# davrempe/contact-human-dynamics

Measured on NVIDIA H100. Metric: optimised frames/sec (batched phys-optim), higher is better.
Workload: dtype f64

## Files before the change

contact-human-dynamics_b200/csrc/chd_api.cu:

```cuda
#include <cuda_runtime.h>

#include <cstdio>
#include <cstdlib>
#include <cstring>
#include <vector>

#include "../../include/chd.h"
#include "chd_dev.h"

__global__ void chd_k_stage_begin(ChdDev D);
__global__ void chd_k_eval(ChdDev D);
__global__ void chd_k_init(ChdDev D);
__global__ void chd_k_kkt(ChdDev D);
__global__ void chd_k_kkt_gwin(ChdDev D);
__global__ void chd_k_kcopy(ChdDev D);
__global__ void chd_k_curv(ChdDev D);
__global__ void chd_k_asm(ChdDev D);
__global__ void chd_k_fp64_peak(int mode, int iters, double* sink);
__global__ void chd_k_hess_base(ChdDev D);
__global__ void chd_k_hess_dur(ChdDev D);
__global__ void chd_k_hess_zero(ChdDev D);
__global__ void chd_k_hess_fin(ChdDev D, int mode);
__global__ void chd_k_tables(ChdDev D);
__global__ void chd_k_clear_dyn(ChdDev D);
// ... 257 lines not shown
    CHD_CUDA(cudaGetDevice(&dev_id));
    CHD_CUDA(cudaDeviceGetDefaultMemPool(&pool, dev_id));
    unsigned long long keep = ~0ull;
    CHD_CUDA(cudaMemPoolSetAttribute(pool, cudaMemPoolAttrReleaseThreshold, &keep));
  }
  CHD_CUDA(cudaStreamCreateWithFlags(&b->copy_stream, cudaStreamNonBlocking));
  CHD_CUDA(cudaEventCreateWithFlags(&b->ev_kkt, cudaEventDisableTiming));
  CHD_CUDA(cudaEventCreateWithFlags(&b->ev_copy, cudaEventDisableTiming));
  CHD_CUDA(cudaEventCreateWithFlags(&b->ev_ls, cudaEventDisableTiming));
  CHD_CUDA(cudaEventCreate(&b->ev0));
  CHD_CUDA(cudaEventCreate(&b->ev1));
#define UP(field) if ((rc = dev_upload(b, hb.field, &D.field))) return rc;
#define UPM(field, T) if ((rc = dev_upload(b, hb.field, (const T**)&D.field))) return rc;
  UP(seq) UPM(poly_T, double) UPM(poly_tend, double) UP(node_const) UP(par) UP(t_dyn) UP(t_rom) UP(t_data) UP(row_lo) UP(row_hi) UP(node_var)
  UP(itab) UP(ent_ptr) UPM(ent_col, int) UP(ent_row) UP(col_ptr) UP(col_ent) UP(var_kkt) UP(row_kkt) UP(row_set) UP(sets) UPM(phase_tend, double)
  UP(dur0) UP(poly_ph)
  if ((rc = dev_upload(b, hb.poly_T, (const double**)&b->poly_T0))) return rc;
  if ((rc = dev_upload(b, hb.poly_tend, (const double**)&b->poly_tend0))) return rc;
  if ((rc = dev_upload(b, hb.phase_tend, (const double**)&b->phase_tend0))) return rc;
  if ((rc = dev_upload(b, hb.ent_col, (const int**)&b->ent_col0))) return rc;
  if ((rc = dev_upload(b, hb.poly_T, (const double**)&D.poly_Tt))) return rc;
  if ((rc = dev_upload(b, hb.poly_tend, (const double**)&D.poly_tendt))) return rc;
#undef UPM
#undef UP
  const size_t B = hb.B, nm = B * hb.n_max, mm = B * hb.m_max;
#define AL(field, cnt) if ((rc = dev_alloc(b, (cnt), &D.field))) return rc;
  AL(x, nm) AL(xt, nm) AL(jty, nm) AL(unobs, nm) AL(dx, nm) AL(grad, nm) AL(g, mm) AL(gt, mm) AL(Jv, B * hb.slots_max) AL(rflag, mm)
  AL(sc, mm) AL(dL, mm) AL(dU, mm) AL(s, mm) AL(y, mm) AL(zL, mm) AL(zU, mm) AL(ds, mm) AL(dy, mm) AL(dzL, mm) AL(dzU, mm)
  int dev = 0, sms = 0, smem_max = 0;
  CHD_CUDA(cudaGetDevice(&dev));
  CHD_CUDA(cudaDeviceGetAttribute(&sms, cudaDevAttrMultiProcessorCount, dev));
// ... 125 lines not shown

int chd_phys_get_layout(const chd_phys_batch* b, int32_t* ent_ptr, int32_t* ent_col, double* row_lo, double* row_hi,
                        int32_t* row_set, int32_t* var_kkt, int32_t* row_kkt) {
  if (!b) return -1;
  const ChdHostBatch& hb = b->hb;
  if (ent_ptr) std::memcpy(ent_ptr, hb.ent_ptr.data(), hb.ent_ptr.size() * sizeof(int));
  if (ent_col) std::memcpy(ent_col, hb.ent_col.data(), hb.ent_col.size() * sizeof(int));
  if (row_lo) std::memcpy(row_lo, hb.row_lo.data(), hb.row_lo.size() * sizeof(double));
  if (row_hi) std::memcpy(row_hi, hb.row_hi.data(), hb.row_hi.size() * sizeof(double));
  if (row_set) std::memcpy(row_set, hb.row_set.data(), hb.row_set.size() * sizeof(int));
  if (var_kkt) std::memcpy(var_kkt, hb.var_kkt.data(), hb.var_kkt.size() * sizeof(int));
  if (row_kkt) std::memcpy(row_kkt, hb.row_kkt.data(), hb.row_kkt.size() * sizeof(int));
  return 0;
}

int chd_phys_get_slot_index(const chd_phys_batch* b, int32_t* ent_row, int32_t* col_ptr, int32_t* col_ent) {
  if (!b) return -1;
  const ChdHostBatch& hb = b->hb;
  if (ent_row) std::memcpy(ent_row, hb.ent_row.data(), hb.ent_row.size() * sizeof(int));
  if (col_ptr) std::memcpy(col_ptr, hb.col_ptr.data(), hb.col_ptr.size() * sizeof(int));
  if (col_ent) std::memcpy(col_ent, hb.col_ent.data(), hb.col_ent.size() * sizeof(int));
  return 0;
}

int chd_phys_get_ent_col(const chd_phys_batch* b, int32_t* ent_col) {
  if (!b || !ent_col) return -1;
  if (b->host_only) {
    std::memcpy(ent_col, b->hb.ent_col.data(), b->hb.ent_col.size() * sizeof(int));
    return 0;
  }
// ... 139 lines not shown
```

contact-human-dynamics_b200/csrc/chd_dev.h:

```cpp
#pragma once
#include "chd_core.h"
#include "chd_kkt_plan.h"
#include "chd_layout.h"

#define CHD_FILT_MAX 24
#define CHD_THREADS 512
#define CHD_NL_GUARD 1.0
#define CHD_NL_FLOOR 1e-4
#define CHD_UNOBS_EPS 1e-14
#define CHD_DW_UNOBS 1e-4
#define CHD_CURV_MIN 1e-8

#define CHD_ROW_ACTIVE 1
#define CHD_ROW_EQ 2
#define CHD_ROW_HASL 4
#define CHD_ROW_HASU 8
#define CHD_ROW_WARM 16

#define CHD_PH_BEGIN 0
#define CHD_PH_RUN 1
#define CHD_PH_FINISHED 2
struct ChdIpm {
  int status;
  int iter, nfilt, ls_fail, max_iter, n_bounds, m_act, pad0;
// ... 25 lines not shown
  double w_data[3], w_vel[3], w_acc[3], w_dur;
};

struct ChdDev {
  int B, S, Pmax, n_max, m_max, slots_max, sets_max, tab_max, F_max, Kd_max, Kr_max, Na_max, nb_max, w_max, par_stride,
      n_ee_max, fo_max, Ph_max, win_smem, nbc_max, Q, Qfix, nbt, win_tiles, pan_doubles;
  size_t kstride;
  const ChdSeq* seq;
  double *poly_T, *poly_tend;
  const double *node_const, *par, *t_dyn, *t_rom, *t_data, *row_lo, *row_hi, *dur0;
  const int *node_var, *itab, *ent_ptr, *var_kkt, *row_kkt, *row_set, *poly_ph;
  int* ent_col;
  double *poly_Tt, *poly_tendt;
  double* jty;
  const int *ent_row, *col_ptr, *col_ent;
  const ChdSet* sets;
  double* phase_tend;
  double *x, *xt, *dx, *grad;
  double *g, *gt;
  double* Jv;
  int* rflag;
  unsigned char* unobs;
  double *sc, *dL, *dU, *s, *y, *zL, *zU, *ds, *dy, *dzL, *dzU;
  double* cost;
  double* Kwork;
  double* Kbase;
  double* sol;
  double* scratch;
  double *rhs0, *rhs1;
  size_t scratch_stride;
// ... 55 lines not shown
```

contact-human-dynamics_b200/csrc/chd_kkt.cu:

```cuda
#include <cuda_runtime.h>

#include "chd_block.cuh"
#include "chd_eval.cuh"
#include "chd_kkt_tiles.cuh"

__device__ __forceinline__ void chd_hess_sample(const ChdCtx& c, const ChdKT& K, const int* vk, int s, const ChdSpl* P, const double* sign, int np,
                                                int deriv, double wgt, int lane, double* ws) {
  const bool tau = c.opt_dur && s >= 2 && deriv == 0;
  if (lane < 28) {
    const int pa = lane / 14, q = lane % 14;
    double v0 = 0.0, v1 = 0.0, v2 = 0.0;
    int ia = -1;
    if (pa < np) {
      if (q < 12) {
        const int va = P[pa].var[q];
        const double wa = sign[pa] * chd_slot_w(P[pa], deriv, q);
        if (va >= 0 && wa != 0.0) {
          ia = vk[va];
          v0 = q % 3 == 0 ? wa : 0.0, v1 = q % 3 == 1 ? wa : 0.0, v2 = q % 3 == 2 ? wa : 0.0;
        }
      } else if (tau) {
        ChdTau u;
        chd_spl_tau(c, s, s - 2, P[pa], u);
        const int var = q == 12 ? u.va : u.vb;
// ... 7 lines not shown
  const int ne = np * 14;
  for (int idx = lane; idx < ne * ne; idx += 32) {
    const int a = idx / ne, bq = idx - a * ne;
    const int ia = (int)ws[a * 4], ib = (int)ws[bq * 4];
    if (ia < 0 || ib < 0 || ia < ib) continue;
    const double v = ws[a * 4 + 1] * ws[bq * 4 + 1] + ws[a * 4 + 2] * ws[bq * 4 + 2] + ws[a * 4 + 3] * ws[bq * 4 + 3];
    if (v != 0.0) chd_kadd(K, ia, ib, wgt * v);
  }
  __syncwarp();
}

__device__ void chd_hess_build(const ChdDev& D, int b, const ChdStageDev& sg, double* base, int part, int nparts) {
  const int tid = threadIdx.x, nt = blockDim.x;
  const ChdSeq* h = D.seq + b;
  ChdKT K;
  chd_kt_init(D, h, base, K);
  K.ovf = &D.ipm[b].band_ovf;
  const double sf = D.ipm[b].sf;
  const int* vk = D.var_kkt + (size_t)b * D.n_max;
  ChdCtx c;
  chd_make_ctx(D, b, D.x + (size_t)b * D.n_max, c);
  c.dyn = D.ipm[b].dyn;
  c.opt_dur = sg.opt_dur;
  const int n_ee = h->n_ee, nsp = 2 + n_ee, F = h->F, ns = h->n_smooth;
  __shared__ double s_hws[CHD_THREADS / 32][28 * 4];
  const int lane = tid & 31, warp = tid >> 5, nwarp = nt >> 5;
  for (int it = part * nwarp + warp; it < nsp * F; it += nparts * nwarp) {
    const int s = it / F, i = it % F, cls = s < 2 ? s : 2;
    ChdSpl P[2];
    double sgn[2] = {1.0, -1.0};
    chd_spl_at(c, s, c.t_data[i], P[1]);
// ... 42 lines not shown
}
__global__ void __launch_bounds__(128) chd_k_hess_fin(ChdDev D, int mode) {
  const int b = blockIdx.x;
  ChdIpm& I = D.ipm[b];
  double* base;
  if (mode == 0) {
    if (I.phase != CHD_PH_BEGIN) return;
    base = D.Kbase + (size_t)b * D.kstride;
  } else {
    if (I.phase != CHD_PH_RUN || !I.kw_req || !D.stages[I.stage].opt_dur) return;
    base = D.Kwork + (size_t)b * D.kstride;
  }
  const ChdSeq* h = D.seq + b;
  const int* vk = D.var_kkt + (size_t)b * D.n_max;
  ChdKT K;
  chd_kt_init(D, h, base, K);
  unsigned char* un = D.unobs + (size_t)b * D.n_max;
  const int mot_lo = h->sp_xoff[2], mot_hi = h->sp_xoff[2 + h->n_ee];
  for (int i = mot_lo + threadIdx.x; i < mot_hi; i += blockDim.x) {
    const int k = vk[i];
    un[i] = k >= 0 && *chd_kdiag(K, k) <= CHD_UNOBS_EPS;
  }
  __syncthreads();
  if (mode == 0 && threadIdx.x == 0) I.phase = CHD_PH_RUN;
}

__device__ __forceinline__ void chd_curv_rows(const ChdDev& D, int b, const ChdKT& K, const ChdStageDev& sg, int wid, int nw, int lane,
                                              double* ws) {
  const ChdSeq* h = D.seq + b;
  const size_t ro = (size_t)b * D.m_max, vo = (size_t)b * D.n_max;
  const int* vk = D.var_kkt + vo;
// ... 81 lines not shown
}

__global__ void __launch_bounds__(256) chd_k_hess_zero(ChdDev D) {
  const int b = blockIdx.y;
  if (D.ipm[b].phase != CHD_PH_BEGIN) return;
  chd_hess_clear(D, b, D.Kbase + (size_t)b * D.kstride, blockIdx.x, gridDim.x);
  chd_hess_clear(D, b, D.Kwork + (size_t)b * D.kstride, blockIdx.x, gridDim.x);
  if (blockIdx.x == 0) chd_rhs_clear(D, b);
}
__global__ void __launch_bounds__(256, 2) chd_k_hess_base(ChdDev D) {
  __shared__ double s_ws[8][192];
  const int b = blockIdx.y;
  if (D.ipm[b].phase != CHD_PH_BEGIN) return;
  const ChdStageDev sg = D.stages[D.ipm[b].stage];
  ChdKT K;
  chd_kt_init(D, D.seq + b, D.Kwork + (size_t)b * D.kstride, K);
  K.ovf = &D.ipm[b].band_ovf;
  const int warp = threadIdx.x >> 5, nwarp = blockDim.x >> 5;
  chd_curv_rows(D, b, K, sg, blockIdx.x * nwarp + warp, gridDim.x * nwarp, threadIdx.x & 31, s_ws[warp]);
  chd_hess_build(D, b, sg, D.Kbase + (size_t)b * D.kstride, blockIdx.x, gridDim.x);
  chd_hess_build(D, b, sg, D.Kwork + (size_t)b * D.kstride, blockIdx.x, gridDim.x);
}

__device__ __forceinline__ void chd_assemble(const ChdDev& D, int b, const ChdKT& K, double delta_w, double sf, int t0, int tstep,
                                             double* g0, double* g1) {
  const ChdSeq* h = D.seq + b;
  const int n = D.stages[D.ipm[b].stage].opt_dur ? h->n : h->n - h->n_dur;
  const int m = h->m, Na = K.Na;
  const size_t ro = (size_t)b * D.m_max, vo = (size_t)b * D.n_max;
  const int* rf = D.rflag + ro;
  const int* vk = D.var_kkt + vo;
// ... 97 lines not shown
  const int b = blockIdx.x;
  c.b = b, c.I = &I;
  c.sg = D.stages[I.stage];
  const ChdSeq* h = c.h = D.seq + b;
  c.n = h->n, c.m = h->m, c.tid = threadIdx.x, c.nt = blockDim.x;
  c.lane = c.tid & 31, c.warp = c.tid >> 5, c.nwarp = c.nt >> 5;
  c.ro = (size_t)b * D.m_max, c.vo = (size_t)b * D.n_max;
  c.rf = D.rflag + c.ro;
  c.vk = D.var_kkt + c.vo;
  c.rk = D.row_kkt + c.ro;
  c.ep = D.ent_ptr + (size_t)b * (D.m_max + 1);
  c.ec = D.ent_col + (size_t)b * D.slots_max;
  c.Jv = D.Jv + (size_t)b * D.slots_max;
  c.grad = D.grad + c.vo;
  ChdKT& K = c.K;
  chd_kt_init(D, h, D.Kwork + (size_t)b * D.kstride, K);
  K.ovf = &I.band_ovf;
  if (!c.sg.opt_dur) K.q = D.Qfix - 1;
  c.n_act = c.sg.opt_dur ? c.n : c.n - h->n_dur;
  c.Qs = K.Q, c.Q = c.sg.opt_dur ? K.Q : D.Qfix, c.nbt = K.nbt, c.nbp8 = K.nbp8, c.nbl = c.sg.opt_dur ? h->nb : h->nb_fix, c.nbc = K.nbc;
  c.NBR = c.nbl, c.nbt_s = (c.nbl + 1 + 7) >> 3;
  c.n_even = (size_t)((D.n_max + 1) & ~1), c.xs_len = (size_t)(8 * D.nbc_max + c.nbp8);
  double* gs = WS ? nullptr : D.scratch + (size_t)b * D.scratch_stride;
  c.red = sm;
  c.cc = c.red + CHD_KKT_THREADS;
  c.ypan = c.cc + c.nbp8 * c.nbp8;
  c.xpan = c.ypan + (c.Q + c.nbt) * 64;
  c.dinv = c.ypan + D.pan_doubles;
  c.win_region = (size_t)D.win_tiles * 64 + (size_t)c.Qs * c.nbt * 64;
  c.win = WS ? c.dinv + 16 : gs + c.n_even + c.xs_len + 8 * (size_t)D.nbc_max;
  c.bwin = c.win + (size_t)D.win_tiles * 64;
  c.vecn = WS ? c.win + c.win_region - c.n_even : gs;
  c.xs = WS ? c.vecn - c.xs_len : c.vecn + c.n_even;
// ... 248 lines not shown
        tl[i].C[r8] = c0[i], tl[i].C[r8 + 1] = c1[i];
      }
  }
}

template <bool WS>
__device__ __forceinline__ void chd_kkt_factor(const ChdKktCtx& c, int& s_fail) {
  const ChdKT& K = c.K;
  const int tid = c.tid, nt = c.nt, lane = c.lane, warp = c.warp, nwarp = c.nwarp;
  const int Qs = c.Qs, Q = c.Q, nbt = c.nbt, nbp8 = c.nbp8, nbc = c.nbc, nbt_s = c.nbt_s;
  double *cc = c.cc, *ypan = c.ypan, *xpan = c.xpan, *dinv = c.dinv, *win = c.win, *bwin = c.bwin;
  for (int i = tid; i < nbp8 * nbp8; i += nt) cc[i] = K.corn[i];
  if (WS) {
    for (int idx = tid; idx < Q * Q * 64; idx += nt) {
      const int e = idx & 63, pr = idx >> 6, J = pr / Q, t = pr % Q;
      if (J + t < Q && J < nbc && J + t < nbc) win[chd_win_slot(J + t, J, Q) * 64 + e] = K.band[((size_t)J * Qs + t) * 64 + e];
    }
    for (int idx = tid; idx < Q * nbt * 64; idx += nt) {
      const int J = idx / (nbt * 64);
      if (J < nbc) bwin[idx] = K.bord[(size_t)J * nbt * 64 + idx % (nbt * 64)];
    }
  }
  __syncthreads();
  __shared__ int s_rs[2][96];
  __shared__ int s_gnz[2][96];
  constexpr int kPairs = WS ? 3000 : CHD_KKT_GROUPS_MAX * (CHD_KKT_GROUPS_MAX + 1) / 2;
  __shared__ unsigned short s_pairs[kPairs];
  __shared__ unsigned char s_cmp[CHD_KKT_THREADS / 32][64];
  __shared__ __align__(16) double s_winv[2][64];
  const int GB = K.q, Gm = K.q + nbt_s, npairs = Gm * (Gm + 1) / 2;
  for (int p = tid; p < npairs && p < kPairs; p += nt) {
    int gi = (int)((sqrt(8.0 * p + 1.0) - 1.0) * 0.5);
    while (gi * (gi + 1) / 2 > p) --gi;
    while ((gi + 1) * (gi + 2) / 2 <= p) ++gi;
    s_pairs[p] = (unsigned short)((gi << 8) | (p - gi * (gi + 1) / 2));
  }
  auto tri = [](int a_, int b_) { return a_ > b_ ? a_ * (a_ + 1) / 2 + b_ : b_ * (b_ + 1) / 2 + a_; };
  for (int g = tid; g < GB; g += nt) s_rs[0][g] = (1 + g) % Q;
  for (int g = tid; g < 96; g += nt) s_gnz[0][g] = 0, s_gnz[1][g] = 0;
  if (warp == 0) {
    const bool ok = chd_tile_ldl(WS ? win : K.band, dinv, s_winv[0], lane);
    if (!ok && lane == 0) s_fail = 1;
  }
  __syncthreads();
  int kslot = 0, cur = 0;
  for (int Kc = 0; Kc < nbc; ++Kc, cur ^= 1) {
    const int tq = min(K.q, nbc - 1 - Kc);
    const int* rs = s_rs[cur];
    auto band_tile = [&](int gi, int gj) -> double* {
      return WS ? win + (size_t)tri(rs[gi], rs[gj]) * 64 : K.band + ((size_t)(Kc + 1 + gj) * Qs + (gi - gj)) * 64;
    };
    auto bord_tile = [&](int bi, int gj) -> double* {
      return WS ? bwin + ((size_t)rs[gj] * nbt + bi) * 64 : K.bord + ((size_t)(Kc + 1 + gj) * nbt + bi) * 64;
    };
    double* Tkk = WS ? win + (size_t)tri(kslot, kslot) * 64 : K.band + (size_t)Kc * Qs * 64;
    double* Bk = WS ? bwin + (size_t)kslot * nbt * 64 : K.bord + (size_t)Kc * nbt * 64;
    const double* dv = dinv + 8 * cur;
    {
      const double* wv = s_winv[cur];
      const int r = lane >> 2, k = lane & 3;
      const double2 wf = *reinterpret_cast<const double2*>(wv + 2 * lane);
      const double d0 = dv[2 * k], d1 = dv[2 * k + 1];
// ... 11 lines not shown
                     : "+d"(c0), "+d"(c1)
                     : "d"(ay), "d"(wf.y));
        const double x0 = c0 * d0, x1 = c1 * d1;
        ypan[pg * 64 + f0] = c0, ypan[pg * 64 + f1] = c1;
        xpan[pg * 64 + f0] = x0, xpan[pg * 64 + f1] = x1;
        double* G = band_t ? K.band + ((size_t)Kc * Qs + 1 + g) * 64 : K.bord + ((size_t)Kc * nbt + (g - tq)) * 64;
        *reinterpret_cast<double2*>(G + r * 8 + 2 * k) = make_double2(x0, x1);
        const bool nz = __any_sync(0xffffffffu, x0 != 0.0 || x1 != 0.0);
        if (lane == 0 && nz) s_gnz[cur][pg] = 1;
      }
    }
    if (WS)
      for (int e = tid; e < 64; e += nt) K.band[(size_t)Kc * Qs * 64 + e] = Tkk[e];
    __syncthreads();
    const int In = Kc + Q;
    if (WS && In < nbc) {
      for (int idx = tid - 32; idx < Q * 32 + nbt_s * 32; idx += nt - 32) {
        if (idx < 0) break;
        const int tile = idx >> 5, off = (idx & 31) * 2;
        if (tile < Q) {
          const int J = tile < GB ? Kc + 1 + tile : In;
          double* dst = tile < GB ? win + (size_t)tri(kslot, rs[tile]) * 64 : Tkk;
          chd_copy16(dst + off, K.band + ((size_t)J * Qs + (In - J)) * 64 + off, WS);
        } else {
          chd_copy16(Bk + (tile - Q) * 64 + off, K.bord + (size_t)In * nbt * 64 + (tile - Q) * 64 + off, WS);
        }
      }
    }
    if (warp == 0) {
      if (tq >= 1) {
        double* Tn = band_tile(0, 0);
        chd_tile_sub_xyT(Tn, xpan, ypan, lane);
        __syncwarp();
        const bool ok = chd_tile_ldl(Tn, dinv + 8 * (cur ^ 1), s_winv[cur ^ 1], lane);
        if (!ok && lane == 0) s_fail = 1;
      }
    } else {
      if (warp == 1) {
        for (int g = lane; g < GB; g += 32) {
          int v = kslot + 2 + g;
          while (v >= Q) v -= Q;
          s_rs[cur ^ 1][g] = v;
        }
        for (int g = lane; g < Gm; g += 32) s_gnz[cur ^ 1][g] = 0;
      }
      if (!WS && Gm > 64) chd_kkt_update_wide(c, s_pairs, s_gnz[cur], GB, npairs, tq, band_tile, bord_tile);
      else chd_kkt_update_compact(c, s_pairs, s_cmp[warp], s_gnz[cur], GB, Gm, tq, band_tile, bord_tile);
    }
// ... 47 lines not shown
    const double* bt = K.bord + (size_t)(i >> 3) * nbt * 64 + (i & 7);
    double v = bt[NBR * 8];
    for (int q2 = 0; q2 < nbl; ++q2) v -= bt[q2 * 8] * xb[q2];
    accv[i] = v;
  }
  const int per = Q * 64;
  const int R = max(1, (int)((c.win_region - (WS ? c.n_even + c.xs_len : 0)) / 64) / (2 * Q));
  double* stg = c.win;
  auto stage_chunk = [&](int Ktop, int buf, int t0, int tstep) {
    for (int idx = t0; idx < R * Q * 32; idx += tstep) {
      const int rr = idx / (Q * 32), rem = idx - rr * (Q * 32);
      const int Kr = Ktop - rr;
      if (Kr < 0) break;
      const int tile = rem >> 5, off = (rem & 31) * 2;
      const int J = tile == 0 ? Kr : Kr - tile;
      if (J < 0) continue;
      chd_copy16(stg + ((size_t)buf * R + rr) * per + tile * 64 + off, K.band + ((size_t)J * Qs + (Kr - J)) * 64 + off, WS);
    }
  };
  stage_chunk(nbc - 1, 0, tid, nt);
  chd_copy_wait(WS);
  __syncthreads();
  int buf = 0;
  for (int Ktop = nbc - 1; Ktop >= 0; Ktop -= R, buf ^= 1) {
    if (warp != 0) {
      stage_chunk(Ktop - R, buf ^ 1, tid - 32, nt - 32);
    } else {
      for (int rr = 0; rr < R && Ktop - rr >= 0; ++rr) {
        const int Kc = Ktop - rr;
        const double* T0 = stg + ((size_t)buf * R + rr) * per;
        double xk[8];
#pragma unroll
        for (int cl = 7; cl >= 0; --cl) {
          double v = accv[Kc * 8 + cl];
#pragma unroll
          for (int p = 7; p > cl; --p) v -= T0[p * 8 + cl] * xk[p];
          xk[cl] = v;
        }
        if (lane < 8) {
          const int gi = Kc * 8 + lane;
          double v = xk[0];
#pragma unroll
          for (int cl = 1; cl < 8; ++cl) v = lane == cl ? xk[cl] : v;
          xs[gi] = v;
          if (gi < Na) sol[gi] = v;
        }
        const int nrow = min(K.q, Kc);
        for (int idx = lane; idx < nrow * 8; idx += 32) {
          const int g = idx >> 3, cl = idx & 7;
          const double* T = T0 + (g + 1) * 64;
          double v = 0.0;
#pragma unroll
          for (int r = 0; r < 8; ++r) v += T[r * 8 + cl] * xk[r];
          accv[(Kc - 1 - g) * 8 + cl] -= v;
        }
        __syncwarp();
      }
    }
    chd_copy_wait(WS);
    __syncthreads();
  }
}
// ... 120 lines not shown
}
#undef CHD_PROF

__global__ void __launch_bounds__(256) chd_k_kcopy(ChdDev D) {
  const int b = blockIdx.y;
  if (!D.ipm[b].kw_req) return;
  if (blockIdx.x == 0) chd_rhs_clear(D, b);
  if (D.stages[D.ipm[b].stage].opt_dur && D.ipm[b].phase == CHD_PH_RUN) {
    chd_hess_clear(D, b, D.Kwork + (size_t)b * D.kstride, blockIdx.x, gridDim.x);
    return;
  }
  const size_t cnt2 = D.kstride / 2, per = (cnt2 + gridDim.x - 1) / gridDim.x;
  const size_t lo = (size_t)blockIdx.x * per, hi = lo + per < cnt2 ? lo + per : cnt2;
  const double2* src = reinterpret_cast<const double2*>(D.Kbase + (size_t)b * D.kstride);
  double2* dst = reinterpret_cast<double2*>(D.Kwork + (size_t)b * D.kstride);
  const size_t nt = blockDim.x;
  size_t i = lo + threadIdx.x;
  for (; i + 3 * nt < hi; i += 4 * nt) {
    const double2 v0 = src[i], v1 = src[i + nt], v2 = src[i + 2 * nt], v3 = src[i + 3 * nt];
    dst[i] = v0, dst[i + nt] = v1, dst[i + 2 * nt] = v2, dst[i + 3 * nt] = v3;
  }
  for (; i < hi; i += nt) dst[i] = src[i];
}

__global__ void __launch_bounds__(256) chd_k_curv(ChdDev D) {
  __shared__ double s_ws[8 * 192];
  const int b = blockIdx.y;
  const ChdIpm& I = D.ipm[b];
  if (!I.kw_req || I.phase != CHD_PH_RUN) return;
  ChdKT K;
  chd_kt_init(D, D.seq + b, D.Kwork + (size_t)b * D.kstride, K);
  K.ovf = &D.ipm[b].band_ovf;
  const int warp = threadIdx.x >> 5, lane = threadIdx.x & 31;
  chd_curv_rows(D, b, K, D.stages[I.stage], blockIdx.x * 8 + warp, gridDim.x * 8, lane, s_ws + warp * 192);
}

__global__ void __launch_bounds__(256) chd_k_asm(ChdDev D) {
  const int b = blockIdx.y;
  const ChdIpm& I = D.ipm[b];
  if (I.phase != CHD_PH_RUN) return;
  ChdKT K;
  chd_kt_init(D, D.seq + b, D.Kwork + (size_t)b * D.kstride, K);
  K.ovf = &D.ipm[b].band_ovf;
  if (!D.stages[I.stage].opt_dur) K.q = D.Qfix - 1;
  const size_t go = (size_t)b * (D.Na_max + D.nb_max);
  chd_assemble(D, b, K, I.delta_w, I.sf, blockIdx.x * blockDim.x + threadIdx.x, gridDim.x * blockDim.x, D.rhs0 + go, D.rhs1 + go);
}

__global__ void __launch_bounds__(256) chd_k_fp64_peak(int mode, int iters, double* sink) {
  const double s = 1.0 + 1e-9 * threadIdx.x;
  double a[8];
#pragma unroll
  for (int i = 0; i < 8; ++i) a[i] = 0.5 + i;
  if (mode == 0) {
    for (int it = 0; it < iters; ++it) {
#pragma unroll
      for (int i = 0; i < 8; ++i) a[i] = fma(a[i], s, 1e-3);
    }
  } else {
// ... 18 lines not shown
```

contact-human-dynamics_b200/csrc/chd_kkt_tiles.cuh:

```cuda
#pragma once
#include "chd_dev.h"

struct ChdKT {
  int Na, Np, nbc, q, Q, nbt, nbp8;
  double *band, *bord, *corn;
  int* ovf;
};

__device__ __forceinline__ void chd_kt_init(const ChdDev& D, const ChdSeq* h, double* base, ChdKT& K) {
  K.Na = h->Na;
  K.Np = (h->Na + 7) & ~7;
  K.nbc = K.Np >> 3;
  K.Q = D.Q;
  K.q = D.Q - 1;
  K.nbt = D.nbt;
  K.nbp8 = 8 * D.nbt;
  K.ovf = nullptr;
  K.band = base;
  K.bord = base + (size_t)D.nbc_max * D.Q * 64;
  K.corn = K.bord + (size_t)D.nbc_max * D.nbt * 64;
}

__device__ __forceinline__ void chd_kadd(const ChdKT& K, int i, int j, double v) {
  if (i < j) { int t = i; i = j; j = t; }
  if (i < K.Na) {
    const int J = j >> 3;
    if ((i >> 3) - J > K.q) {
      if (K.ovf) *K.ovf = 1;
      return;
    }
    atomicAdd(K.band + ((size_t)J * K.Q + ((i >> 3) - J)) * 64 + (i & 7) * 8 + (j & 7), v);
  } else if (j < K.Na) {
    const int b = i - K.Na;
    atomicAdd(K.bord + ((size_t)(j >> 3) * K.nbt + (b >> 3)) * 64 + (b & 7) * 8 + (j & 7), v);
  } else {
    atomicAdd(K.corn + (size_t)(i - K.Na) * K.nbp8 + (j - K.Na), v);
  }
}
__device__ __forceinline__ double* chd_kdiag(const ChdKT& K, int k, bool band = false) {
  if (band || k < K.Na) return K.band + ((size_t)(k >> 3) * K.Q) * 64 + (k & 7) * 9;
  return K.corn + (size_t)(k - K.Na) * (K.nbp8 + 1);
}
// ... 81 lines not shown
```

contact-human-dynamics_b200/csrc/chd_layout.cpp:

```cpp
#include "chd_layout.h"
#include "chd_dev.h"

#include <algorithm>
#include <atomic>
#include <thread>
#include <cmath>
#include <cstring>
#include <numeric>

namespace {

struct PolyInfo {
  int phase, poly_in_phase, n_polys;
  bool constant;
};

struct SplineBuild {
  std::vector<double> T;
  std::vector<int> var;
  std::vector<double> cval;
  std::vector<PolyInfo> info;
  std::vector<char> const_node;
  int xoff = 0, nvar = 0;
  int npoly() const { return (int)T.size(); }
// ... 35 lines not shown
    if (node > 0 && s.info[node - 1].constant) c = true;
    if (node < nn - 1 && s.info[node].constant) c = true;
    s.const_node[node] = c;
  }
  s.var.assign((size_t)nn * 6, -1);
  s.cval.assign((size_t)nn * 6, 0.0);
}

struct SeqBuild {
  ChdSeq h;
  std::vector<SplineBuild> sp;
  std::vector<double> x0, t_dyn, t_rom, t_data, row_lo, row_hi, var_t0, var_t1, row_t;
  std::vector<char> var_fixed, var_stance, var_dur;
  std::vector<ChdSet> sets;
  std::vector<int> itab, ent_ptr, ent_col, var_kkt, row_kkt, row_set;
};

std::vector<double> discretize(double T, double dt) {
  std::vector<double> d = {0.0};
  double t = 0.0;
  for (int i = 0; i < std::floor(T / dt); ++i) {
    t += dt;
    d.push_back(t);
  }
  d.push_back(T);
  return d;
}

bool kkt_fits(int w_max, int nb_max) {
  return chd_kkt_gwin_status(w_max, nb_max, CHD_KKT_GWIN_STATIC_MAX, CHD_SMEM_OPTIN) == CHD_KKT_FITS;
// ... 398 lines not shown
    }
    auto explicit_row = [&](int r) { return sb.row_lo[r] == sb.row_hi[r] || sb.ent_ptr[r + 1] - sb.ent_ptr[r] > 16; };
    for (int r = 0; r < h.m; ++r)
      if (explicit_row(r)) keys.push_back({sb.row_t[r] + 1e-6, 1, r});
    std::stable_sort(keys.begin(), keys.end(), [](const Key& a, const Key& b) { return a.t < b.t; });
    for (size_t i = 0; i < keys.size(); ++i) (keys[i].kind == 0 ? sb.var_kkt[keys[i].id] : sb.row_kkt[keys[i].id]) = (int)i;
    h.Na = (int)keys.size();
    h.nb_fix = (int)border.size();
    if (!h.dur_band)
      for (int v = 0; v < h.n; ++v)
        if (sb.var_dur[v]) border.push_back(v);
    h.nb = (int)border.size();
    for (int j = 0; j < h.nb; ++j) sb.var_kkt[border[j]] = h.Na + j;
    int w = 0, w_fix = 0;
    bool with_ext = true;
    auto span = [&](const int* cols, int cnt, int rowpos) {
      int lo = 1 << 30, hi = -1;
      for (int i = 0; i < cnt; ++i) {
        if (cols[i] < 0) continue;
        if (!with_ext && sb.var_dur[cols[i]]) continue;
        int k = sb.var_kkt[cols[i]];
        if (k < 0 || k >= h.Na) continue;
        lo = std::min(lo, k), hi = std::max(hi, k);
      }
      if (rowpos >= 0) lo = std::min(lo, rowpos), hi = std::max(hi, rowpos);
      if (hi >= 0) (with_ext ? w : w_fix) = std::max(with_ext ? w : w_fix, hi - lo);
    };
    auto clique = [&](const std::vector<int>& cols) { span(cols.data(), (int)cols.size(), -1); };
    const std::vector<std::vector<int>> no_opts;
    std::vector<int> merged;
    for (int pass = 0; pass < 2; ++pass)
    for (int r = 0; r < h.m; ++r) {
      with_ext = pass == 1;
      merged.assign(sb.ent_col.begin() + sb.ent_ptr[r], sb.ent_col.begin() + sb.ent_ptr[r + 1]);
      if (with_ext) merged.insert(merged.end(), row_ext[r].begin(), row_ext[r].end());
      const std::vector<std::vector<int>>& opts = with_ext ? row_tau[r] : no_opts;
      const int* c = merged.data();
      const int cnt = (int)merged.size();
      if (sb.row_kkt[r] >= 0) {
        for (int i = 0; i < cnt; ++i) span(c + i, 1, sb.row_kkt[r]);
        for (const auto& o : opts)
// ... 14 lines not shown
        for (int q = 0; q < 12; ++q) cols.push_back(sb.sp[s].var[poly * 6 + q]);
        if (with_ext) ext_nodes(s, poly, sb.t_data[i], cols);
        if (with_ext && s >= 2) tau_reach(s - 2, sb.t_data[i], opts);
        if (i < h.n_smooth) {
          int poly2 = chd_locate(tend[s].data(), sb.sp[s].npoly(), sb.t_data[i] + p.dt, &tl);
          for (int q = 0; q < 12; ++q) cols.push_back(sb.sp[s].var[poly2 * 6 + q]);
          if (with_ext) ext_nodes(s, poly2, sb.t_data[i] + p.dt, cols);
          if (with_ext && s >= 2) tau_reach(s - 2, sb.t_data[i] + p.dt, opts);
        }
        for_options(cols, opts, clique);
      }
    }
    w = std::max(w, w_fix);
    h.w = w;
    h.w_fix = w_fix;
    const double grp = (w_fix + 7) / 8 + 1 + (h.nb_fix + 1 + 7) / 8;
    return (double)((h.Na + 7) / 8) * grp * grp;
  };
  const double cand[4] = {0.15, 0.35, 0.5, 1e30};
  int best = 0;
  double best_cost = 0;
  for (int ci = 0; ci < 4; ++ci) {
    const double cst = order_kkt(cand[ci]);
    if (ci == 0 || cst < 0.9 * best_cost) best = ci, best_cost = cst;
  }
  order_kkt(cand[best]);
  if (h.dur_band && !kkt_fits(h.w, h.nb)) return 1;
  return 0;
}

// ... 125 lines not shown
      int* cent = hb.col_ent.data() + (size_t)i * hb.slots_max;
      for (int r = 0; r < sb.h.m; ++r)
        for (int e = sb.ent_ptr[r]; e < sb.ent_ptr[r + 1]; ++e) erow[e] = r;
      std::vector<int> cnt(hb.n_max + 1, 0);
      for (int e = 0; e < sb.h.nslots; ++e)
        if (sb.ent_col[e] >= 0) cnt[sb.ent_col[e] + 1]++;
      for (int v = 0; v < hb.n_max; ++v) cnt[v + 1] += cnt[v];
      std::copy(cnt.begin(), cnt.end(), cptr);
      for (int e = 0; e < sb.h.nslots; ++e)
        if (sb.ent_col[e] >= 0) cent[cnt[sb.ent_col[e]]++] = e;
    }
    std::copy(sb.var_kkt.begin(), sb.var_kkt.end(), hb.var_kkt.begin() + (size_t)i * hb.n_max);
    std::copy(sb.row_kkt.begin(), sb.row_kkt.end(), hb.row_kkt.begin() + (size_t)i * hb.m_max);
    std::copy(sb.sets.begin(), sb.sets.end(), hb.sets.begin() + (size_t)i * hb.sets_max);
  }
  const unsigned ACC = CHD_MASK(CHD_SET_ACC), LEG = CHD_MASK(CHD_SET_TERRAIN) | CHD_MASK(CHD_SET_ROM),
                 HEEL = CHD_MASK(CHD_SET_HEEL), DYN = CHD_MASK(CHD_SET_DYN) | CHD_MASK(CHD_SET_FORCE),
                 HGT = CHD_MASK(CHD_SET_HEIGHT);
  ChdStageCfg s1 = {ACC, {1.0, 1.0, 1.0}, {0.1, 0.1, 0.1}, {0, 0, 0}, 7000, 0.0};
  ChdStageCfg s2 = {ACC | LEG | DYN | HEEL, {wt.w_com_lin, wt.w_com_ang, wt.w_ee}, {0.001, 0.001, wt.w_smooth},
                    {0.0001, 0.0001, 0.0001}, 7000, 0.0};
  hb.stage[CHD_STAGE_11] = s1;
  hb.stage[CHD_STAGE_12] = s1;
  hb.stage[CHD_STAGE_12].set_mask = ACC | LEG | HEEL;
  hb.stage[CHD_STAGE_21] = s2;
  hb.stage[CHD_STAGE_22] = s2;
  hb.stage[CHD_STAGE_22].set_mask |= HGT;
  hb.stage[CHD_STAGE_22].max_iter = 2500;
  hb.stage[CHD_STAGE_3] = hb.stage[CHD_STAGE_22];
  hb.stage[CHD_STAGE_3].set_mask |= CHD_MASK(CHD_SET_TOTTIME) | CHD_MASK(CHD_SET_DURPOS);
// ... 8 lines not shown
```

contact-human-dynamics_b200/csrc/chd_layout.h:

```cpp
#pragma once
#include <vector>

#include "../../include/chd.h"
#include "chd_core.h"

struct ChdStageCfg {
  unsigned set_mask;
  double w_data[3];
  double w_vel[3];
  double w_acc[3];
  int max_iter;
  double w_dur;
};

struct ChdHostBatch {
  int B = 0;
  int S = 0, Pmax = 0, n_max = 0, m_max = 0, slots_max = 0, sets_max = 0, tab_max = 0, F_max = 0, Kd_max = 0, Kr_max = 0;
  int Na_max = 0, nb_max = 0, w_max = 0, w_fix_max = 0, n_ee_max = 0, fo_max = 0, Ph_max = 0;
  std::vector<ChdSeq> seq;
  std::vector<double> poly_T, poly_tend, node_const, par, t_dyn, t_rom, t_data, row_lo, row_hi, x0, phase_tend;
  std::vector<double> dur0;
  std::vector<int> node_var, itab, ent_ptr, ent_col, var_kkt, row_kkt, row_set;
  std::vector<int> poly_ph;
  std::vector<int> ent_row, col_ptr, col_ent;
  std::vector<ChdSet> sets;
  ChdStageCfg stage[6];
  int par_stride() const { return (18 + 3 * n_ee_max) * F_max; }
};

int chd_build_layout(const chd_phys_problem* problems, int batch, const chd_phys_weights& w, ChdHostBatch& out,
                     int stage3_band_above = -1);
```

contact-human-dynamics_b200/phys.py:

```python
from __future__ import annotations

import ctypes as C
import os
from typing import List, Optional, Sequence

import numpy as np

from .io_formats import PhysProblem

_HERE = os.path.dirname(os.path.abspath(__file__))
_LIB = None

STAGES = {"1.1": 0, "1.2": 1, "2.1": 2, "2.2": 3, "3": 4, "4": 5}
SET_NAMES = {0: "acc", 1: "terrain", 2: "rom", 3: "dyn", 4: "force", 5: "heel", 6: "height", 7: "tottime", 8: "durpos"}


class _Problem(C.Structure):
    _fields_ = [("n_frames", C.c_int32), ("n_ee", C.c_int32), ("dt", C.c_double),
                ("hip_left", C.POINTER(C.c_double)), ("hip_right", C.POINTER(C.c_double)),
                ("max_leg_length", C.c_double), ("max_heel_length", C.c_double), ("heel_dist", C.c_double),
                ("body_mass", C.c_double), ("inertia", C.POINTER(C.c_double)), ("base_lin", C.POINTER(C.c_double)),
                ("base_ang", C.POINTER(C.c_double)), ("ee_pos", C.POINTER(C.c_double)),
                ("floor_normal", C.c_double * 3), ("floor_point", C.c_double * 3),
                ("ee_start_contact", C.POINTER(C.c_int32)), ("ee_n_phases", C.POINTER(C.c_int32)),
# ... 16 lines not shown

_vp, _i32, _i64, _int, _f64 = C.c_void_p, C.c_int32, C.c_int64, C.c_int, C.c_double

SIGNATURES = {
    "chd_phys_batch_create": (_int, [C.POINTER(_Problem), _i32, C.POINTER(_Weights), _i32, C.POINTER(_Options),
                                     C.POINTER(_vp)]),
    "chd_phys_batch_destroy": (None, [_vp]),
    "chd_phys_get_dims": (_int, [_vp, C.POINTER(_Dims)]),
    "chd_phys_get_sizes": (_int, [_vp, _vp]),
    "chd_phys_get_sizes_fixed": (_int, [_vp, _vp]),
    "chd_phys_get_x": (_int, [_vp, _vp]),
    "chd_phys_set_x": (_int, [_vp, _vp]),
    "chd_phys_eval": (_int, [_vp, _i32, _vp, _vp, _vp, _vp]),
    "chd_phys_get_layout": (_int, [_vp] * 8),
    "chd_phys_get_slot_index": (_int, [_vp] * 4),
    "chd_phys_get_ent_col": (_int, [_vp, _vp]),
    "chd_phys_get_duals": (_int, [_vp] * 7),
    "chd_phys_stage_stats": (_int, [_vp, _vp]),
    "chd_phys_solve_stage": (_int, [_vp, _i32, _i32, _vp, _vp, _vp]),
    "chd_phys_solve": (_int, [_vp] * 6),
    "chd_phys_sample": (_int, [_vp, _vp, _vp]),
    "chd_phys_sample_device": (_int, [_vp, _vp, _vp]),
    "chd_phys_launch_count": (_i64, [_vp]),
    "chd_phys_h2d_bytes": (_i64, [_vp]),
    "chd_phys_reset": (_int, [_vp]),
    "chd_phys_kernel_times": (_int, [_vp, _vp, _vp, _int]),
    "chd_phys_set_timing": (_int, [_vp, _int]),
    "chd_contact_create": (_int, [_vp, _vp, _vp, C.c_float, _i32, C.POINTER(_vp)]),
    "chd_contact_destroy": (None, [_vp]),
    "chd_contact_forward": (_int, [_vp, _vp, _i32, _i32, _vp, _vp, _vp, _vp]),
# ... 132 lines not shown
    def layout(self) -> dict:
        B, d = self.B, self.dims
        out = dict(ent_ptr=np.zeros((B, d["m_max"] + 1), np.int32), ent_col=np.zeros((B, d["slots_max"]), np.int32),
                   row_lo=np.zeros((B, d["m_max"])), row_hi=np.zeros((B, d["m_max"])),
                   row_set=np.zeros((B, d["m_max"]), np.int32), var_kkt=np.zeros((B, d["n_max"]), np.int32),
                   row_kkt=np.zeros((B, d["m_max"]), np.int32))
        self._chk(self.L.chd_phys_get_layout(self.h, *[_ptr(out[k]) for k in ("ent_ptr", "ent_col", "row_lo", "row_hi",
                                                                              "row_set", "var_kkt", "row_kkt")]))
        return out

    def sizes_fixed(self) -> np.ndarray:
        out = np.zeros((self.B, 3), np.int32)
        self._chk(self.L.chd_phys_get_sizes_fixed(self.h, _ptr(out)))
        return out

    def ent_col(self) -> np.ndarray:
        out = np.zeros((self.B, self.dims["slots_max"]), np.int32)
        self._chk(self.L.chd_phys_get_ent_col(self.h, _ptr(out)))
        return out

    def duals(self) -> dict:
        B, d = self.B, self.dims
        out = {k: np.zeros((B, d["m_max"])) for k in ("y", "zL", "zU", "s", "row_scale")}
        out["obj_scale"] = np.zeros(B)
        self._chk(self.L.chd_phys_get_duals(self.h, *[_ptr(out[k]) for k in ("y", "zL", "zU", "s", "row_scale", "obj_scale")]))
        return out

    def stage_stats(self) -> np.ndarray:
        out = np.zeros((6, self.B, 4))
        self._chk(self.L.chd_phys_stage_stats(self.h, _ptr(out)))
# ... 103 lines not shown
```

include/chd.h:

```cpp
#ifndef CHD_H_
#define CHD_H_
#include <stdint.h>

#ifdef __cplusplus
extern "C" {
#endif

typedef struct chd_phys_problem {
  int32_t n_frames;
  int32_t n_ee;
  double dt;
  const double* hip_left;
  const double* hip_right;
  double max_leg_length, max_heel_length, heel_dist, body_mass;
  const double* inertia;
  const double* base_lin;
  const double* base_ang;
  const double* ee_pos;
  double floor_normal[3], floor_point[3];
  const int32_t* ee_start_contact;
  const int32_t* ee_n_phases;
  const double* ee_durations;
} chd_phys_problem;

// ... 15 lines not shown
int chd_phys_batch_create(const chd_phys_problem* problems, int32_t batch, const chd_phys_weights* weights,
                          int32_t device, const chd_phys_options* opt, chd_phys_batch** out);
void chd_phys_batch_destroy(chd_phys_batch* b);
int chd_phys_get_dims(const chd_phys_batch* b, chd_phys_dims* dims);
int chd_phys_get_sizes(const chd_phys_batch* b, int32_t* sizes6);
int chd_phys_get_sizes_fixed(const chd_phys_batch* b, int32_t* sizes3);

int chd_phys_get_x(const chd_phys_batch* b, double* x_host);
int chd_phys_set_x(chd_phys_batch* b, const double* x_host);

int chd_phys_eval(chd_phys_batch* b, int32_t stage, double* cost, double* grad, double* g, double* jac_vals);

int chd_phys_get_layout(const chd_phys_batch* b, int32_t* ent_ptr, int32_t* ent_col, double* row_lo, double* row_hi,
                        int32_t* row_set, int32_t* var_kkt, int32_t* row_kkt);
int chd_phys_get_slot_index(const chd_phys_batch* b, int32_t* ent_row, int32_t* col_ptr, int32_t* col_ent);

int chd_phys_get_ent_col(const chd_phys_batch* b, int32_t* ent_col);
int chd_phys_get_duals(const chd_phys_batch* b, double* y, double* zL, double* zU, double* s, double* row_scale,
                       double* obj_scale);
int chd_phys_stage_stats(const chd_phys_batch* b, double* stats);

int chd_phys_solve_stage(chd_phys_batch* b, int32_t stage, int32_t max_iter, int32_t* status, int32_t* iters,
                         double* stats);

int chd_phys_solve(chd_phys_batch* b, double* samples, int32_t* frames_out, int32_t* success,
                   int32_t* stage_status, int32_t* stage_iters);

int chd_phys_sample(chd_phys_batch* b, double* out, int32_t* frames_out);

int chd_phys_sample_device(chd_phys_batch* b, double* out_device, void* stream);
// ... 50 lines not shown
```

Baseline: 13260.

## Use per-column skyline profile for banded KKT factorization instead of uniform bandwidth

New measurement: 13620 (median of 6 runs). 2.7% higher.

```diff
diff --git a/contact-human-dynamics_b200/csrc/chd_api.cu b/contact-human-dynamics_b200/csrc/chd_api.cu
--- a/contact-human-dynamics_b200/csrc/chd_api.cu
+++ b/contact-human-dynamics_b200/csrc/chd_api.cu
@@ -295,7 +295,7 @@
 #define UPM(field, T) if ((rc = dev_upload(b, hb.field, (const T**)&D.field))) return rc;
   UP(seq) UPM(poly_T, double) UPM(poly_tend, double) UP(node_const) UP(par) UP(t_dyn) UP(t_rom) UP(t_data) UP(row_lo) UP(row_hi) UP(node_var)
   UP(itab) UP(ent_ptr) UPM(ent_col, int) UP(ent_row) UP(col_ptr) UP(col_ent) UP(var_kkt) UP(row_kkt) UP(row_set) UP(sets) UPM(phase_tend, double)
-  UP(dur0) UP(poly_ph)
+  UP(dur0) UP(poly_ph) UP(kkt_prof)
   if ((rc = dev_upload(b, hb.poly_T, (const double**)&b->poly_T0))) return rc;
   if ((rc = dev_upload(b, hb.poly_tend, (const double**)&b->poly_tend0))) return rc;
   if ((rc = dev_upload(b, hb.phase_tend, (const double**)&b->phase_tend0))) return rc;
@@ -451,6 +451,12 @@
   return 0;
 }
 
+int chd_phys_get_kkt_profile(const chd_phys_batch* b, int32_t* prof) {
+  if (!b || !prof) return -1;
+  std::memcpy(prof, b->hb.kkt_prof.data(), b->hb.kkt_prof.size() * sizeof(int));
+  return 0;
+}
+
 int chd_phys_get_slot_index(const chd_phys_batch* b, int32_t* ent_row, int32_t* col_ptr, int32_t* col_ent) {
   if (!b) return -1;
   const ChdHostBatch& hb = b->hb;
diff --git a/contact-human-dynamics_b200/csrc/chd_dev.h b/contact-human-dynamics_b200/csrc/chd_dev.h
--- a/contact-human-dynamics_b200/csrc/chd_dev.h
+++ b/contact-human-dynamics_b200/csrc/chd_dev.h
@@ -63,6 +63,7 @@
   double *poly_Tt, *poly_tendt;
   double* jty;
   const int *ent_row, *col_ptr, *col_ent;
+  const int* kkt_prof;
   const ChdSet* sets;
   double* phase_tend;
   double *x, *xt, *dx, *grad;
diff --git a/contact-human-dynamics_b200/csrc/chd_kkt.cu b/contact-human-dynamics_b200/csrc/chd_kkt.cu
--- a/contact-human-dynamics_b200/csrc/chd_kkt.cu
+++ b/contact-human-dynamics_b200/csrc/chd_kkt.cu
@@ -45,7 +45,7 @@
   const int tid = threadIdx.x, nt = blockDim.x;
   const ChdSeq* h = D.seq + b;
   ChdKT K;
-  chd_kt_init(D, h, base, K);
+  chd_kt_init(D, b, base, K);
   K.ovf = &D.ipm[b].band_ovf;
   const double sf = D.ipm[b].sf;
   const int* vk = D.var_kkt + (size_t)b * D.n_max;
@@ -118,7 +118,7 @@
   const ChdSeq* h = D.seq + b;
   const int* vk = D.var_kkt + (size_t)b * D.n_max;
   ChdKT K;
-  chd_kt_init(D, h, base, K);
+  chd_kt_init(D, b, base, K);
   unsigned char* un = D.unobs + (size_t)b * D.n_max;
   const int mot_lo = h->sp_xoff[2], mot_hi = h->sp_xoff[2 + h->n_ee];
   for (int i = mot_lo + threadIdx.x; i < mot_hi; i += blockDim.x) {
@@ -230,7 +230,7 @@
   if (D.ipm[b].phase != CHD_PH_BEGIN) return;
   const ChdStageDev sg = D.stages[D.ipm[b].stage];
   ChdKT K;
-  chd_kt_init(D, D.seq + b, D.Kwork + (size_t)b * D.kstride, K);
+  chd_kt_init(D, b, D.Kwork + (size_t)b * D.kstride, K);
   K.ovf = &D.ipm[b].band_ovf;
   const int warp = threadIdx.x >> 5, nwarp = blockDim.x >> 5;
   chd_curv_rows(D, b, K, sg, blockIdx.x * nwarp + warp, gridDim.x * nwarp, threadIdx.x & 31, s_ws[warp]);
@@ -358,9 +358,8 @@
   c.Jv = D.Jv + (size_t)b * D.slots_max;
   c.grad = D.grad + c.vo;
   ChdKT& K = c.K;
-  chd_kt_init(D, h, D.Kwork + (size_t)b * D.kstride, K);
+  chd_kt_init(D, b, D.Kwork + (size_t)b * D.kstride, K);
   K.ovf = &I.band_ovf;
-  if (!c.sg.opt_dur) K.q = D.Qfix - 1;
   c.n_act = c.sg.opt_dur ? c.n : c.n - h->n_dur;
   c.Qs = K.Q, c.Q = c.sg.opt_dur ? K.Q : D.Qfix, c.nbt = K.nbt, c.nbp8 = K.nbp8, c.nbl = c.sg.opt_dur ? h->nb : h->nb_fix, c.nbc = K.nbc;
   c.NBR = c.nbl, c.nbt_s = (c.nbl + 1 + 7) >> 3;
@@ -639,7 +638,8 @@
   if (WS) {
     for (int idx = tid; idx < Q * Q * 64; idx += nt) {
       const int e = idx & 63, pr = idx >> 6, J = pr / Q, t = pr % Q;
-      if (J + t < Q && J < nbc && J + t < nbc) win[chd_win_slot(J + t, J, Q) * 64 + e] = K.band[((size_t)J * Qs + t) * 64 + e];
+      if (J + t < Q && J < nbc && J + t < nbc && chd_kt_first(K, J + t) <= J)
+        win[chd_win_slot(J + t, J, Q) * 64 + e] = K.band[((size_t)J * Qs + t) * 64 + e];
     }
     for (int idx = tid; idx < Q * nbt * 64; idx += nt) {
       const int J = idx / (nbt * 64);
@@ -670,7 +670,7 @@
   __syncthreads();
   int kslot = 0, cur = 0;
   for (int Kc = 0; Kc < nbc; ++Kc, cur ^= 1) {
-    const int tq = min(K.q, nbc - 1 - Kc);
+    const int tq = chd_kt_last(K, Kc) - Kc;
     const int* rs = s_rs[cur];
     auto band_tile = [&](int gi, int gj) -> double* {
       return WS ? win + (size_t)tri(rs[gi], rs[gj]) * 64 : K.band + ((size_t)(Kc + 1 + gj) * Qs + (gi - gj)) * 64;
@@ -712,9 +712,9 @@
       for (int e = tid; e < 64; e += nt) K.band[(size_t)Kc * Qs * 64 + e] = Tkk[e];
     __syncthreads();
     const int In = Kc + Q;
-    if (WS && In < nbc) {
-      for (int idx = tid - 32; idx < Q * 32 + nbt_s * 32; idx += nt - 32) {
-        if (idx < 0) break;
+    if (WS && In < nbc && warp != 0) {
+      const int i0 = 32 * (chd_kt_first(K, In) - (Kc + 1));
+      for (int idx = i0 + tid - 32; idx < Q * 32 + nbt_s * 32; idx += nt - 32) {
         const int tile = idx >> 5, off = (idx & 31) * 2;
         if (tile < Q) {
           const int J = tile < GB ? Kc + 1 + tile : In;
@@ -726,10 +726,12 @@
       }
     }
     if (warp == 0) {
-      if (tq >= 1) {
+      if (Kc + 1 < nbc) {
         double* Tn = band_tile(0, 0);
-        chd_tile_sub_xyT(Tn, xpan, ypan, lane);
-        __syncwarp();
+        if (tq >= 1) {
+          chd_tile_sub_xyT(Tn, xpan, ypan, lane);
+          __syncwarp();
+        }
         const bool ok = chd_tile_ldl(Tn, dinv + 8 * (cur ^ 1), s_winv[cur ^ 1], lane);
         if (!ok && lane == 0) s_fail = 1;
       }
@@ -807,7 +809,7 @@
       if (Kr < 0) break;
       const int tile = rem >> 5, off = (rem & 31) * 2;
       const int J = tile == 0 ? Kr : Kr - tile;
-      if (J < 0) continue;
+      if (J < chd_kt_first(K, Kr)) continue;
       chd_copy16(stg + ((size_t)buf * R + rr) * per + tile * 64 + off, K.band + ((size_t)J * Qs + (Kr - J)) * 64 + off, WS);
     }
   };
@@ -838,7 +840,7 @@
           xs[gi] = v;
           if (gi < Na) sol[gi] = v;
         }
-        const int nrow = min(K.q, Kc);
+        const int nrow = Kc - chd_kt_first(K, Kc);
         for (int idx = lane; idx < nrow * 8; idx += 32) {
           const int g = idx >> 3, cl = idx & 7;
           const double* T = T0 + (g + 1) * 64;
@@ -989,22 +991,40 @@
   const size_t lo = (size_t)blockIdx.x * per, hi = lo + per < cnt2 ? lo + per : cnt2;
   const double2* src = reinterpret_cast<const double2*>(D.Kbase + (size_t)b * D.kstride);
   double2* dst = reinterpret_cast<double2*>(D.Kwork + (size_t)b * D.kstride);
+  ChdKT K;
+  chd_kt_init(D, b, D.Kbase + (size_t)b * D.kstride, K);
+  const int col2 = D.Q * 32;
+  const size_t band2 = (size_t)D.nbc_max * col2;
+  auto live = [&](size_t i) {
+    if (i >= band2) return true;
+    const int J = (int)(i / col2);
+    return J < K.nbc && (int)(i - (size_t)J * col2) < (chd_kt_last(K, J) - J + 1) * 32;
+  };
   const size_t nt = blockDim.x;
   size_t i = lo + threadIdx.x;
   for (; i + 3 * nt < hi; i += 4 * nt) {
-    const double2 v0 = src[i], v1 = src[i + nt], v2 = src[i + 2 * nt], v3 = src[i + 3 * nt];
-    dst[i] = v0, dst[i + nt] = v1, dst[i + 2 * nt] = v2, dst[i + 3 * nt] = v3;
-  }
-  for (; i < hi; i += nt) dst[i] = src[i];
-}
-
-__global__ void __launch_bounds__(256) chd_k_curv(ChdDev D) {
+    const bool l0 = live(i), l1 = live(i + nt), l2 = live(i + 2 * nt), l3 = live(i + 3 * nt);
+    double2 v0, v1, v2, v3;
+    if (l0) v0 = src[i];
+    if (l1) v1 = src[i + nt];
+    if (l2) v2 = src[i + 2 * nt];
+    if (l3) v3 = src[i + 3 * nt];
+    if (l0) dst[i] = v0;
+    if (l1) dst[i + nt] = v1;
+    if (l2) dst[i + 2 * nt] = v2;
+    if (l3) dst[i + 3 * nt] = v3;
+  }
+  for (; i < hi; i += nt)
+    if (live(i)) dst[i] = src[i];
+}
+
+__global__ void __launch_bounds__(256, 2) chd_k_curv(ChdDev D) {
   __shared__ double s_ws[8 * 192];
   const int b = blockIdx.y;
   const ChdIpm& I = D.ipm[b];
   if (!I.kw_req || I.phase != CHD_PH_RUN) return;
   ChdKT K;
-  chd_kt_init(D, D.seq + b, D.Kwork + (size_t)b * D.kstride, K);
+  chd_kt_init(D, b, D.Kwork + (size_t)b * D.kstride, K);
   K.ovf = &D.ipm[b].band_ovf;
   const int warp = threadIdx.x >> 5, lane = threadIdx.x & 31;
   chd_curv_rows(D, b, K, D.stages[I.stage], blockIdx.x * 8 + warp, gridDim.x * 8, lane, s_ws + warp * 192);
@@ -1015,9 +1035,8 @@
   const ChdIpm& I = D.ipm[b];
   if (I.phase != CHD_PH_RUN) return;
   ChdKT K;
-  chd_kt_init(D, D.seq + b, D.Kwork + (size_t)b * D.kstride, K);
+  chd_kt_init(D, b, D.Kwork + (size_t)b * D.kstride, K);
   K.ovf = &D.ipm[b].band_ovf;
-  if (!D.stages[I.stage].opt_dur) K.q = D.Qfix - 1;
   const size_t go = (size_t)b * (D.Na_max + D.nb_max);
   chd_assemble(D, b, K, I.delta_w, I.sf, blockIdx.x * blockDim.x + threadIdx.x, gridDim.x * blockDim.x, D.rhs0 + go, D.rhs1 + go);
 }
diff --git a/contact-human-dynamics_b200/csrc/chd_kkt_tiles.cuh b/contact-human-dynamics_b200/csrc/chd_kkt_tiles.cuh
--- a/contact-human-dynamics_b200/csrc/chd_kkt_tiles.cuh
+++ b/contact-human-dynamics_b200/csrc/chd_kkt_tiles.cuh
@@ -4,28 +4,35 @@
 struct ChdKT {
   int Na, Np, nbc, q, Q, nbt, nbp8;
   double *band, *bord, *corn;
+  const int* prof;
   int* ovf;
 };
 
-__device__ __forceinline__ void chd_kt_init(const ChdDev& D, const ChdSeq* h, double* base, ChdKT& K) {
+__device__ __forceinline__ void chd_kt_init(const ChdDev& D, int b, double* base, ChdKT& K) {
+  const ChdSeq* h = D.seq + b;
+  const ChdIpm& I = D.ipm[b];
+  const int s3 = D.stages[I.stage].opt_dur;
   K.Na = h->Na;
   K.Np = (h->Na + 7) & ~7;
   K.nbc = K.Np >> 3;
   K.Q = D.Q;
-  K.q = D.Q - 1;
+  K.q = s3 ? D.Q - 1 : D.Qfix - 1;
   K.nbt = D.nbt;
   K.nbp8 = 8 * D.nbt;
+  K.prof = D.kkt_prof + ((size_t)b * 3 + (s3 ? 1 : (I.dyn ? 2 : 0))) * 2 * D.nbc_max;
   K.ovf = nullptr;
   K.band = base;
   K.bord = base + (size_t)D.nbc_max * D.Q * 64;
   K.corn = K.bord + (size_t)D.nbc_max * D.nbt * 64;
 }
+__device__ __forceinline__ int chd_kt_first(const ChdKT& K, int I) { return __ldg(K.prof + 2 * I); }
+__device__ __forceinline__ int chd_kt_last(const ChdKT& K, int J) { return __ldg(K.prof + 2 * J + 1); }
 
 __device__ __forceinline__ void chd_kadd(const ChdKT& K, int i, int j, double v) {
   if (i < j) { int t = i; i = j; j = t; }
   if (i < K.Na) {
     const int J = j >> 3;
-    if ((i >> 3) - J > K.q) {
+    if (J < chd_kt_first(K, i >> 3)) {
       if (K.ovf) *K.ovf = 1;
       return;
     }
diff --git a/contact-human-dynamics_b200/csrc/chd_layout.cpp b/contact-human-dynamics_b200/csrc/chd_layout.cpp
--- a/contact-human-dynamics_b200/csrc/chd_layout.cpp
+++ b/contact-human-dynamics_b200/csrc/chd_layout.cpp
@@ -73,6 +73,7 @@
   std::vector<char> var_fixed, var_stance, var_dur;
   std::vector<ChdSet> sets;
   std::vector<int> itab, ent_ptr, ent_col, var_kkt, row_kkt, row_set;
+  std::vector<int> prof[2];
 };
 
 std::vector<double> discretize(double T, double dt) {
@@ -501,17 +502,32 @@
     for (int j = 0; j < h.nb; ++j) sb.var_kkt[border[j]] = h.Na + j;
     int w = 0, w_fix = 0;
     bool with_ext = true;
+    const int nbc = (h.Na + 7) / 8;
+    for (auto& pr : sb.prof) {
+      pr.resize(nbc);
+      std::iota(pr.begin(), pr.end(), 0);
+    }
     auto span = [&](const int* cols, int cnt, int rowpos) {
       int lo = 1 << 30, hi = -1;
+      auto member = [&](int i) {
+        if (cols[i] < 0) return -1;
+        if (!with_ext && sb.var_dur[cols[i]]) return -1;
+        const int k = sb.var_kkt[cols[i]];
+        return k < h.Na ? k : -1;
+      };
       for (int i = 0; i < cnt; ++i) {
-        if (cols[i] < 0) continue;
-        if (!with_ext && sb.var_dur[cols[i]]) continue;
-        int k = sb.var_kkt[cols[i]];
-        if (k < 0 || k >= h.Na) continue;
-        lo = std::min(lo, k), hi = std::max(hi, k);
+        const int k = member(i);
+        if (k >= 0) lo = std::min(lo, k), hi = std::max(hi, k);
       }
       if (rowpos >= 0) lo = std::min(lo, rowpos), hi = std::max(hi, rowpos);
-      if (hi >= 0) (with_ext ? w : w_fix) = std::max(with_ext ? w : w_fix, hi - lo);
+      if (hi < 0) return;
+      (with_ext ? w : w_fix) = std::max(with_ext ? w : w_fix, hi - lo);
+      std::vector<int>& pr = sb.prof[with_ext];
+      for (int i = 0; i < cnt; ++i) {
+        const int k = member(i);
+        if (k >= 0) pr[k >> 3] = std::min(pr[k >> 3], lo >> 3);
+      }
+      if (rowpos >= 0) pr[rowpos >> 3] = std::min(pr[rowpos >> 3], lo >> 3);
     };
     auto clique = [&](const std::vector<int>& cols) { span(cols.data(), (int)cols.size(), -1); };
     const std::vector<std::vector<int>> no_opts;
@@ -556,6 +572,9 @@
     w = std::max(w, w_fix);
     h.w = w;
     h.w_fix = w_fix;
+    for (int J = 0; J < nbc; ++J) sb.prof[1][J] = std::min(sb.prof[1][J], sb.prof[0][J]);
+    for (auto& pr : sb.prof)
+      for (int J = nbc - 2; J >= 0; --J) pr[J] = std::min(pr[J], pr[J + 1]);
     const double grp = (w_fix + 7) / 8 + 1 + (h.nb_fix + 1 + 7) / 8;
     return (double)((h.Na + 7) / 8) * grp * grp;
   };
@@ -711,6 +730,22 @@
     std::copy(sb.row_kkt.begin(), sb.row_kkt.end(), hb.row_kkt.begin() + (size_t)i * hb.m_max);
     std::copy(sb.sets.begin(), sb.sets.end(), hb.sets.begin() + (size_t)i * hb.sets_max);
   }
+  {
+    const ChdKktPlan P = chd_kkt_plan(hb.Na_max, hb.nb_max, hb.w_max, hb.w_fix_max, hb.n_max, 0, 0, CHD_SMEM_OPTIN);
+    const int nbc_max = P.nbc_max;
+    hb.kkt_prof.assign((size_t)B * 3 * nbc_max * 2, 0);
+    for (int i = 0; i < B; ++i)
+      for (int s = 0; s < 3; ++s) {
+        const std::vector<int>& pr = sbs[i].prof[s != 0];
+        const int q = (s == 1 ? P.Q : P.Qfix) - 1, nbc = (int)pr.size();
+        int* t = hb.kkt_prof.data() + ((size_t)i * 3 + s) * nbc_max * 2;
+        for (int J = 0; J < nbc_max; ++J) t[2 * J] = J < nbc ? std::max(pr[J], J - q) : J, t[2 * J + 1] = J;
+        for (int J = 0, Jr = 0; J < nbc; ++J) {
+          while (Jr + 1 < nbc && t[2 * (Jr + 1)] <= J) ++Jr;
+          t[2 * J + 1] = Jr;
+        }
+      }
+  }
   const unsigned ACC = CHD_MASK(CHD_SET_ACC), LEG = CHD_MASK(CHD_SET_TERRAIN) | CHD_MASK(CHD_SET_ROM),
                  HEEL = CHD_MASK(CHD_SET_HEEL), DYN = CHD_MASK(CHD_SET_DYN) | CHD_MASK(CHD_SET_FORCE),
                  HGT = CHD_MASK(CHD_SET_HEIGHT);
diff --git a/contact-human-dynamics_b200/csrc/chd_layout.h b/contact-human-dynamics_b200/csrc/chd_layout.h
--- a/contact-human-dynamics_b200/csrc/chd_layout.h
+++ b/contact-human-dynamics_b200/csrc/chd_layout.h
@@ -23,6 +23,7 @@
   std::vector<int> node_var, itab, ent_ptr, ent_col, var_kkt, row_kkt, row_set;
   std::vector<int> poly_ph;
   std::vector<int> ent_row, col_ptr, col_ent;
+  std::vector<int> kkt_prof;
   std::vector<ChdSet> sets;
   ChdStageCfg stage[6];
   int par_stride() const { return (18 + 3 * n_ee_max) * F_max; }
diff --git a/contact-human-dynamics_b200/phys.py b/contact-human-dynamics_b200/phys.py
--- a/contact-human-dynamics_b200/phys.py
+++ b/contact-human-dynamics_b200/phys.py
@@ -54,6 +54,7 @@
     "chd_phys_eval": (_int, [_vp, _i32, _vp, _vp, _vp, _vp]),
     "chd_phys_get_layout": (_int, [_vp] * 8),
     "chd_phys_get_slot_index": (_int, [_vp] * 4),
+    "chd_phys_get_kkt_profile": (_int, [_vp, _vp]),
     "chd_phys_get_ent_col": (_int, [_vp, _vp]),
     "chd_phys_get_duals": (_int, [_vp] * 7),
     "chd_phys_stage_stats": (_int, [_vp, _vp]),
@@ -216,6 +217,11 @@
         self._chk(self.L.chd_phys_get_sizes_fixed(self.h, _ptr(out)))
         return out
 
+    def kkt_profile(self) -> np.ndarray:
+        out = np.zeros((self.B, 3, (self.dims["na_max"] + 7) // 8, 2), np.int32)
+        self._chk(self.L.chd_phys_get_kkt_profile(self.h, _ptr(out)))
+        return out
+
     def ent_col(self) -> np.ndarray:
         out = np.zeros((self.B, self.dims["slots_max"]), np.int32)
         self._chk(self.L.chd_phys_get_ent_col(self.h, _ptr(out)))
diff --git a/include/chd.h b/include/chd.h
--- a/include/chd.h
+++ b/include/chd.h
@@ -53,6 +53,7 @@
 int chd_phys_get_layout(const chd_phys_batch* b, int32_t* ent_ptr, int32_t* ent_col, double* row_lo, double* row_hi,
                         int32_t* row_set, int32_t* var_kkt, int32_t* row_kkt);
 int chd_phys_get_slot_index(const chd_phys_batch* b, int32_t* ent_row, int32_t* col_ptr, int32_t* col_ent);
+int chd_phys_get_kkt_profile(const chd_phys_batch* b, int32_t* prof);
 
 int chd_phys_get_ent_col(const chd_phys_batch* b, int32_t* ent_col);
 int chd_phys_get_duals(const chd_phys_batch* b, double* y, double* zL, double* zU, double* s, double* row_scale,
```
